# Hydr10n/DirectX-Raytracing-Spheres-Demo

Hardware: AMD Instinct MI355X
Metric: Mrays/s (CastRay-equivalents incl. primaries) at 1920x1080, 8 bounces, 1 spp (higher is better)
Workload: dtype f32

## Files before the change

### directx-raytracing-spheres-demo_amd/csrc/pt_api.hip

```cpp
#include <hip/hip_runtime.h>
#include <rccl/rccl.h>
#include <dlfcn.h>
#include <link.h>

#include <algorithm>
#include <chrono>
#include <cmath>
#include <cstdio>
#include <cstdlib>
#include <cstring>
#include <new>
#include <string>
#include <limits>
#include <vector>

#include "../../include/pt_api.h"
#include "pt_kernels.h"
#include "pt_beam_cache.h"
#include "pt_bloom.h"
#include "pt_nrd.h"
#include "pt_denoise.h"
#include "pt_lbvh.h"
#include "pt_lbvh_gpu.h"

using namespace pt;

namespace {

constexpr uint32_t kMaxLdsBytes = 160u * 1024u;
constexpr uint32_t kSahMaxSpheres = 4096u;
constexpr uint32_t kLdsSceneBudget = 64u * 1024u;

struct EventPair {
    hipEvent_t a, b;
    int kind;
};

}

struct Knobs {
    int split = -1, traverse_blocks_per_cu = -1, fused_threads = -1, no_adaptive_grid = -1, shade_blocks_per_cu = -1, tail_threshold = -1,
        tail_blocks_per_cu = -1, loop_threads = -1, inline2_min_slots = -1, tail_after = -1, seg = -1, loop_use_tail = -1, fuse_loop = -1,
        ray_replacement = -1, dyn_blocks_per_cu = -1, debug_counts = -1, sah = -1, sah_max_spheres = -1, beams = -1, wide = -1, descent = -1, roctx = -1, lane_priority = -1, fused_refit = -1, beam_reach = -1, beam_max_slack_pct = -1, beam_max_margin = -1, beam_share_wgs = -1, refl_beams = -1;
};

struct Lane {
    hipStream_t stream = nullptr;
    hipEvent_t ev_done = nullptr;
    size_t cap_slots = 0;
    RayQueue q[2]{};
    Scratch scratch{};
    bool scratch_spp = false;
    uint32_t* d_counts = nullptr;
    size_t cap_counts = 0;
    uint32_t parity = 0;
    uint32_t* h_counts = nullptr;
    uint32_t* h_prev_counts = nullptr;
    uint32_t* d_prev_counts = nullptr;
    uint64_t prev_signature = 0;
    uint32_t* d_seg_counts = nullptr;
    static constexpr uint32_t kTotals = 10;
    unsigned long long* d_totals = nullptr;
    float4* d_sph = nullptr;
    float4* d_sph_sorted = nullptr;
    float4* d_nodes = nullptr;
    uint32_t* d_refit_flags = nullptr;
    uint32_t* d_refit_hdr = nullptr;
    PtSphere* h_stage = nullptr;
    const float4* d_stage = nullptr;
    hipEvent_t ev_upload = nullptr;
    hipEvent_t ev_poll[4] = {};
    uint32_t scene_n = 0;
    bool scene_private = false;
    uint64_t sph_gen = 0;
    bool needs_refit = false;
    bool upload_pending = false;
    const void* last_out = nullptr;
    const void* last_dn[3] = {};
    const void* last_di[2] = {};
    float4* d_rot = nullptr;
    float4* h_rot_stage = nullptr;
    hipEvent_t ev_rot = nullptr;
    uint64_t rot_gen = 0;
    uint32_t rot_n = 0;
    float4* d_prev_pose = nullptr;
    float4* h_prev_stage = nullptr;
    hipEvent_t ev_prev = nullptr;
    uint32_t prev_cap = 0;
    hipEvent_t ev_gb_in = nullptr;
    void* last_gb[13] = {};
};
constexpr uint32_t kMaxLanes = 8;

struct PtContext {
    int device = 0;
    hipStream_t stream = nullptr;
// ... 364 lines not shown
    sv.nodes = priv ? L->d_nodes : c->d_nodes;
    sv.wide = priv ? nullptr : c->d_wide;
    sv.sph_sorted = priv ? L->d_sph_sorted : c->d_sph_sorted;
    sv.sorted_id = c->d_leaf_ids ? c->d_leaf_ids : c->d_sorted_id;
    sv.alpha_class = c->d_alpha_class;
    sv.alpha_tested = c->alpha_tested ? 1u : 0u;
    sv.sph = priv ? L->d_sph : c->d_sph;
    sv.mats = c->d_mats;
    sv.n = c->n;
    sv.n_nodes = c->n_nodes;
    sv.stack_depth = stack_entries(c, sv.wide != nullptr);
    sv.descent_cap = c->lds_scene ? 0u : knob_or(c->knobs.descent, 8u);
    sv.lds_scene = c->lds_scene ? 1u : 0u;
    for (int i = 0; i < 4; i++) sv.env[i] = c->sd.EnvironmentLightColor[i];
    if (c->has_textures) { sv.tex = c->d_tex; sv.tex_maps = c->d_tex_maps; sv.rot = (c->rot_gen != c->rot_master_gen && L && L->d_rot && L->rot_gen == c->rot_gen) ? L->d_rot : c->d_rot; }
    sv.env_tex = c->sd.EnvironmentLightTextureDescriptor;
    sv.env_cube = c->sd.IsEnvironmentLightTextureCubeMap ? 1u : 0u;
    for (int r = 0; r < 3; r++)
        for (int k = 0; k < 3; k++) sv.env_xf[3 * r + k] = c->sd.EnvironmentLightTransform[4 * r + k];
    sv.lights = c->d_lights; sv.n_lights = c->n_lights;
    return sv;
}

FrameParams make_frame_params(const PtContext* c)
{
    FrameParams fp{};
    fp.cam = camera_params(c->cam, c->gs.RenderSize[0], c->gs.RenderSize[1]);
    fp.frame_index = c->gs.FrameIndex;
    fp.bounces = c->gs.Bounces;
    fp.spp = c->gs.SamplesPerPixel;
    fp.rr_enabled = c->gs.IsRussianRouletteEnabled ? 1u : 0u;
    fp.throughput_threshold = c->gs.ThroughputThreshold;
    fp.inv_spp = 1.0f / (float)c->gs.SamplesPerPixel;
    fp.di_enabled = (c->gs.IsDIEnabled && c->n_lights > 0) ? 1u : 0u;
    return fp;
}

int env_knob(const char* name)
{
    const char* v = std::getenv(name);
    if (!v || !*v) return -1;
    return (int)std::strtoul(v, nullptr, 10);
}

Knobs read_knobs()
{
    Knobs k;
    k.split = env_knob("PT_SPLIT"); k.traverse_blocks_per_cu = env_knob("PT_TRAVERSE_BLOCKS_PER_CU"); k.fused_threads = env_knob("PT_FUSED_THREADS");
    k.no_adaptive_grid = std::getenv("PT_NO_ADAPTIVE_GRID") ? 1 : -1; k.shade_blocks_per_cu = env_knob("PT_SHADE_BLOCKS_PER_CU");
    k.tail_threshold = env_knob("PT_TAIL_THRESHOLD"); k.tail_blocks_per_cu = env_knob("PT_TAIL_BLOCKS_PER_CU"); k.loop_threads = env_knob("PT_LOOP_THREADS");
    k.inline2_min_slots = env_knob("PT_INLINE2_MIN_SLOTS"); k.tail_after = env_knob("PT_TAIL_AFTER"); k.seg = env_knob("PT_SEG");
    k.loop_use_tail = std::getenv("PT_LOOP_USE_TAIL") ? 1 : -1; k.fuse_loop = env_knob("PT_FUSE_LOOP"); k.beam_reach = env_knob("PT_BEAM_REACH"); k.beam_max_slack_pct = env_knob("PT_BEAM_MAX_SLACK_PCT"); k.beam_max_margin = env_knob("PT_BEAM_MAX_MARGIN"); k.beam_share_wgs = env_knob("PT_BEAM_SHARE_WGS"); k.lane_priority = env_knob("PT_LANE_PRIORITY"); k.fused_refit = env_knob("PT_FUSED_REFIT"); k.ray_replacement = env_knob("PT_RAY_REPLACEMENT");
    k.dyn_blocks_per_cu = env_knob("PT_DYN_BLOCKS_PER_CU"); k.debug_counts = std::getenv("PT_DEBUG_COUNTS") ? 1 : -1; k.sah = env_knob("PT_SAH");
    k.sah_max_spheres = env_knob("PT_SAH_MAX_SPHERES"); k.beams = env_knob("PT_BEAMS"); k.refl_beams = env_knob("PT_REFL_BEAMS"); k.wide = env_knob("PT_WIDE"); k.descent = env_knob("PT_DESCENT"); k.roctx = env_knob("PT_ROCTX");
    return k;
}

EventPair* next_events(PtContext* c, int kind)
{
    if (c->ev_used >= (1u << 20)) return nullptr;
    if (c->ev_used == c->ev_pool.size()) {
        EventPair p{};
        if (hipEventCreate(&p.a) != hipSuccess || hipEventCreate(&p.b) != hipSuccess) return nullptr;
        c->ev_pool.push_back(p);
    }
    EventPair* p = &c->ev_pool[c->ev_used++];
    p->kind = kind;
    return p;
}

uint64_t bytes_per_secondary(bool split) { return split ? 144ull : 96ull; }
uint64_t fixed_bytes(bool split, uint64_t slots, uint64_t pixels, uint64_t spp_paths)
{
    return (split ? 112ull * slots : 0ull) + 16ull * pixels + 48ull * spp_paths;
}

FrameCounters make_counters(const Lane& L, uint32_t parity)
{
    FrameCounters fc{};
    fc.counts = L.d_counts + (size_t)parity * 2 * L.cap_counts;
    fc.fold_counts = L.d_counts + (size_t)(parity ^ 1u) * 2 * L.cap_counts;
    fc.n_counts = (uint32_t)L.cap_counts - 1u;
    fc.tail_rays = L.d_totals + 2 + parity;
    fc.fold_tail = L.d_totals + 2 + (parity ^ 1u);
    fc.totals = L.d_totals;
    fc.host_counts = L.d_prev_counts;
    return fc;
}

hipError_t flush_all_counters(Lane& L)
{
    if (!L.d_counts) return hipSuccess;
    for (uint32_t i = 0; i < 2; i++) {
        const FrameCounters fc = make_counters(L, L.parity ^ 1u ^ i);
        hipError_t e = launch_flush_counters(fc.counts, fc.n_counts, fc.tail_rays, fc.totals, fc.host_counts, L.stream);
        if (e != hipSuccess) return e;
    }
    return hipSuccess;
}

void sum_events(PtContext* c, size_t begin, size_t end, PtStats* stats)
{
    for (size_t i = begin; i < end; i++) {
        float t = 0;
        if (hipEventElapsedTime(&t, c->ev_pool[i].a, c->ev_pool[i].b) != hipSuccess) continue;
        switch (c->ev_pool[i].kind) {
            case 2: stats->ms_shade += t; stats->shade_launches++; break;
// ... 312 lines not shown
    c->next_lane = (c->next_lane + 1) % c->n_lanes;
    c->frames++;
    const uint32_t* beam_lists = nullptr;
    const uint32_t* refl_lists = nullptr;
    BeamJob beam_job{};
    if (!split && !L.scene_private && c->n_nodes > 0 && knob_or(c->knobs.beams, 1u) != 0 && std::fabs(c->cam.Jitter[0]) <= 0.5f && std::fabs(c->cam.Jitter[1]) <= 0.5f) {
        hipEvent_t beam_wait = nullptr;
        if ((st = beam_cache_lookup(c, pm, std::min(primary_grid, knob_or(c->knobs.beam_share_wgs, 128u)) * 64u, &beam_lists, &refl_lists, &beam_wait, &beam_job)) != PT_OK) return st;
        if (beam_wait) PT_HIP(c, hipStreamWaitEvent(L.stream, beam_wait, 0));
    } else {
        c->beam.last_key.clear();
        c->beam.inc.active = false;
    }
    if (L.stream != c->stream) {
        const uint64_t nl = c->n_lanes;
        PT_HIP(c, hipEventRecord(c->ev_in[c->calls % nl], c->stream));
        const hipEvent_t marker = c->ev_in[c->calls >= nl - 1 ? (c->calls - (nl - 1)) % nl : 0];
        if (hipEventQuery(marker) != hipSuccess) {
            (void)hipGetLastError();
            PT_HIP(c, hipStreamWaitEvent(L.stream, marker, 0));
        }
        const void* mine[4] = { out, dn ? dn->diffuse : nullptr, dn ? dn->specular : nullptr, dn ? dn->spec_hit_dist : nullptr };
        bool reused = false;
        for (uint32_t i = 0; i < c->n_lanes && !reused; i++) {
            if (&c->lanes[i] == &L) continue;
            const Lane& o = c->lanes[i];
            const void* theirs[6] = { o.last_out, o.last_dn[0], o.last_dn[1], o.last_dn[2], o.last_di[0], o.last_di[1] };
            for (int a = 0; a < 4 && !reused; a++)
                for (int b = 0; b < 6 && !reused; b++) reused = mine[a] && mine[a] == theirs[b];
        }
        if (ext) reused = true;
        if (reused) PT_HIP(c, hipStreamWaitEvent(L.stream, c->ev_in[c->calls % nl], 0));
        L.last_out = out;
        for (int a = 0; a < 3; a++) L.last_dn[a] = mine[a + 1];
        L.last_di[0] = ext ? ext->diffuse : nullptr;
        L.last_di[1] = ext ? ext->specular : nullptr;
        c->calls++;
    }

    const SceneView sv = make_scene_view(c, &L);
    Scratch scr = L.scratch;
    scr.dn = DenoiseOut{};
    if (dn) {
        scr.dn = *dn;
        scr.dn.rec = L.scratch.dn.rec;
        scr.dn.di_s = L.scratch.dn.di_s;
    }
    FrameParams fp = make_frame_params(c);
    if (ext) fp.di_enabled = kDiExternal;
    fp.beam_lists = beam_lists;
    fp.beam_job = beam_job;
    fp.refl_lists = refl_lists;
    L.parity ^= 1u;
    const FrameCounters fc = make_counters(L, L.parity);
    uint32_t* counts = fc.counts;

    const uint64_t signature = ((uint64_t)pm.n_slots << 32) ^ ((uint64_t)bounces << 20) ^ ((uint64_t)spp << 4) ^ pm.mode ^ ((uint64_t)c->n << 40) ^ (split ? 8u : 0u);
    const bool have_prev = spp == 1 && L.prev_signature == signature && L.h_prev_counts[0] == pm.n_slots && c->knobs.no_adaptive_grid < 0;
    auto estimate = [&](size_t k) -> uint32_t {
        if (!have_prev || k >= L.cap_counts) return pm.n_slots;
        const uint64_t e = (uint64_t)L.h_prev_counts[k] + L.h_prev_counts[k] / 4 + 64;
        return (uint32_t)std::min<uint64_t>(e, pm.n_slots);
    };
    const uint32_t trav_cap_wide = c->num_cus * 8u;
    const uint32_t shade_cap = c->num_cus * knob_or(c->knobs.shade_blocks_per_cu, 16);
    const bool loop_is_main = spp > 1 && !split && c->knobs.tail_threshold < 0;
    const uint32_t tail_cap = c->num_cus * knob_or(c->knobs.tail_blocks_per_cu, loop_is_main ? 2 : 8);
    const uint32_t trav_threads = traverse_threads(c->lds_scene);
    const uint32_t loop_threads = knob_or(c->knobs.loop_threads, c->lds_scene && (loop_is_main || big_frame) ? 512u : 256u);
    const bool inline2 = !split && spp == 1 && pm.n_slots >= knob_or(c->knobs.inline2_min_slots, 0u);
    const size_t tail_after = knob_or(c->knobs.tail_after, split ? 4 : (inline2 ? 0 : 1));
    const uint32_t tail_threshold = knob_or(c->knobs.tail_threshold, 262144);

    const bool timed = stats != nullptr;
    const size_t ev_begin = c->ev_used;
    if (timed) PT_HIP(c, hipEventRecord(c->ev0, L.stream));

    auto bracket = [&](int kind, auto&& launch) -> hipError_t {
        EventPair* ev = c->profiling ? next_events(c, kind) : nullptr;
        if (ev) (void)hipEventRecord(ev->a, L.stream);
        hipError_t e = launch();
        if (ev) (void)hipEventRecord(ev->b, L.stream);
        return e;
    };
    auto poll = [&](size_t k, bool& empty, bool& go_loop) -> PtStatus {
        empty = false;
        if (loop_is_main) {
            go_loop = true;
        } else if (spp > 1) {
            constexpr size_t kPollLag = 2;
            PT_HIP(c, hipMemcpyAsync(L.h_counts + k + 1, counts + k + 1, sizeof(uint32_t), hipMemcpyDeviceToHost, L.stream));
            PT_HIP(c, hipEventRecord(L.ev_poll[k & 3], L.stream));
            go_loop = k + 2 >= wf_cap;
            if (k >= kPollLag) {
                PT_HIP(c, hipEventSynchronize(L.ev_poll[(k - kPollLag) & 3]));
                const uint32_t v = L.h_counts[k - kPollLag + 1];
                empty = v == 0;
                go_loop = go_loop || v < tail_threshold;
            }
        } else {
            go_loop = k >= tail_after || k + 2 >= wf_cap;
        }
        return PT_OK;
    };

    auto submit = [&]() -> PtStatus {
        if (ext) {
// ... 1344 lines not shown
```

### directx-raytracing-spheres-demo_amd/csrc/pt_device.h

```cpp
#pragma once

#include <hip/hip_runtime.h>
#include <stdint.h>

#include "pt_bsdf.h"
#include "pt_texture.h"
#include "pt_surface.h"
#include "pt_light.h"

namespace pt {

struct RayQueue {
    float4* q0;
    float4* q1;
    float4* q2;
    uint2* hit;
};

constexpr uint32_t kFlagBounceMask = 0xFFu;
constexpr uint32_t kFlagSampleShift = 8;
constexpr uint32_t kFlagSampleMask = 0xFFFFu;
constexpr uint32_t kFlagDirty = 1u << 24;
constexpr uint32_t kFlagViaTransmission = 1u << 25;
constexpr uint32_t kFlagDnSpecular = 1u << 26;
// ... 73 lines not shown
        const uint32_t bpt_shift = m.ts_shift - 3u;
        const uint32_t b = w >> 6, l = w & 63u;
        const uint32_t lx = ((b & ((1u << bpt_shift) - 1u)) << 3) + (l & 7u), ly = ((b >> bpt_shift) << 3) + (l >> 3);
        uint32_t gt;
        if (m.run == 1u) {
            gt = m.first + k * m.stride;
        } else {
            const uint32_t q = fast_div(k, m.run, m.inv_run, m.exact_div != 0);
            gt = m.first + q * m.stride + (k - q * m.run);
        }
        const uint32_t ty = fast_div(gt, m.tiles_x, m.inv_tiles_x, m.exact_div != 0), tx = gt - ty * m.tiles_x;
        r.px = (tx << m.ts_shift) + lx;
        r.py = (ty << m.ts_shift) + ly;
        r.valid = gt < m.tiles_total && r.px < m.img_w && r.py < m.img_h;
        r.out_index = (k << ts2_shift) + (ly << m.ts_shift) + lx;
    }
    return r;
}

struct BeamJob {
    uint32_t* lists;
    uint32_t first_block, n_blocks;
    float centre[3];
    float slack;
    float right[3], up[3], forward[3];
    float margin_px;
};

struct FrameParams {
    CameraParams cam;
    uint32_t frame_index, bounces, spp, rr_enabled;
    float throughput_threshold;
    float inv_spp;
    uint32_t di_enabled;
    const uint32_t* beam_lists;
    BeamJob beam_job;
    const uint32_t* refl_lists;
};

constexpr uint32_t kDiExternal = 2u;

struct FrameCounters {
    uint32_t* counts;
    uint32_t* fold_counts;
    uint32_t n_counts;
    unsigned long long* tail_rays;
    unsigned long long* fold_tail;
    unsigned long long* totals;
    uint32_t* host_counts;
    uint32_t* seg_counts;
    uint32_t n_segs;
    uint32_t seg_cap;
    uint32_t fuse_loop;
};

constexpr uint32_t kMaxSegs = 2048;

struct DenoiseOut {
    uint32_t mode;
    float4* rec;
    float4* di_s;
    float4* diffuse;
    float4* specular;
    float* spec_hit_dist;
};

struct Scratch {
    float4* sample_rad;
    float4* radiance;
    uint2* primary_hit;
    float4* di;
    float4* primary_cache;
    DenoiseOut dn;
};

}
```

### directx-raytracing-spheres-demo_amd/csrc/pt_trace.h

```cpp
#pragma once

#include "pt_kernels.h"
#include "pt_beam.h"

namespace pt {

__device__ __forceinline__ uint32_t lane_id() { return __builtin_amdgcn_mbcnt_hi(~0u, __builtin_amdgcn_mbcnt_lo(~0u, 0u)); }

__device__ __forceinline__ float fast_rcp(float x) { return __builtin_amdgcn_rcpf(x); }

__device__ __forceinline__ float slab_rcp(float d)
{
    const float kTiny = 1e-30f;
    return fast_rcp(__builtin_fabsf(d) < kTiny ? __builtin_copysignf(kTiny, d) : d);
}

__device__ __forceinline__ void block_atomic_add(unsigned long long* counter, unsigned long long v)
{
    __shared__ unsigned long long s_part[16];
#pragma unroll
    for (int off = 32; off > 0; off >>= 1) v += __shfl_down(v, off, 64);
    __syncthreads();
    if ((threadIdx.x & 63u) == 0) s_part[threadIdx.x >> 6] = v;
    __syncthreads();
// ... 184 lines not shown
                stack[sp] = stack_encode<StackT>(far_c);
                sp += stride;
                node = near_c;
            } else if (h0) {
                node = c0;
            } else if (h1) {
                node = c1;
            } else if (sp == 0) {
                node = kTraversalDone;
            } else {
                sp -= stride;
                node = stack_decode(stack[sp]);
            }
            if (--budget == 0u) break;
        }
        if (node == kTraversalDone) break;
        if (node >= 0) continue;
        {
            if (kCount) n_spheres_tested++;
            const uint32_t k = ~(uint32_t)node;
            const float4 s = sph[k];
            float t;
            if (intersect_sphere(o, d, tmin, kInf, make_f3(s.x, s.y, s.z), s.w, t)) {
                const uint32_t idf = ids[k];
                if ((idf >> kIdClassShift) == 0u || alpha_candidate<kAlphaTex>(sv, idf, make_f3(s.x, s.y, s.z), s.w, o, d, t)) {
                    const uint32_t id = idf & kIdMask;
                    if (t < best || (t == best && best_id != kMissId && id < best_id)) { best = t; best_id = id; }
                }
            }
        }
        if (sp == 0) break;
        sp -= stride;
        node = stack_decode(stack[sp]);
    }
    t_out = best; id_out = best_id;
    if (kCount && visits) { visits[0] += n_nodes_visited; visits[1] += n_spheres_tested; }
}

template <bool kLds, typename StackT, bool kAlphaTex = false>
__device__ __forceinline__ void closest_hit_any(const SceneView& sv, const float4* __restrict__ nodes, const float4* __restrict__ sph,
                                                const uint32_t* __restrict__ ids, f3 o, f3 d, float tmin, float tmax, StackT* stack, uint32_t stride,
                                                float& t_out, uint32_t& id_out, uint32_t* visits = nullptr)
{
    if (!kLds && visits) {
        if (sv.wide) closest_hit<StackT, true, true, kAlphaTex>(sv, sv.wide, sph, ids, sv.n, o, d, tmin, tmax, stack, stride, t_out, id_out, visits, sv.descent_cap);
        else closest_hit<StackT, true, false, kAlphaTex>(sv, nodes, sph, ids, sv.n, o, d, tmin, tmax, stack, stride, t_out, id_out, visits, sv.descent_cap);
    } else if (!kLds && sv.wide) {
        closest_hit<StackT, false, true, kAlphaTex>(sv, sv.wide, sph, ids, sv.n, o, d, tmin, tmax, stack, stride, t_out, id_out, nullptr, sv.descent_cap);
    } else {
        closest_hit<StackT, false, false, kAlphaTex>(sv, nodes, sph, ids, sv.n, o, d, tmin, tmax, stack, stride, t_out, id_out, nullptr, sv.descent_cap);
    }
}

__device__ __forceinline__ void flush_visit_counters(unsigned long long* totals, const uint32_t v[2])
{
    block_atomic_add(totals + 6, v[0]);
    block_atomic_add(totals + 7, v[1]);
}


template <typename StackT>
__device__ __forceinline__ void beam_walk_block(const SceneView& sv, const float4* nodes, const uint32_t* ids, StackT* stack, uint32_t stride, const PixelMap& pm,
                                                const CameraParams& cam, float slack, float margin_px, uint32_t tile, uint32_t* __restrict__ lists)
{
    uint32_t* rec = lists + (size_t)tile * kBeamRecord;
    const PixelRef pr = slot_to_pixel(pm, tile << 6);
    uint32_t count = 0;
    if (pr.valid) {
        const Beam b = make_beam(cam, pr.px, pr.py, slack, margin_px);
        if (sv.n == 1) {
            rec[1] = ids[0];
            count = 1;
        } else {
            int node = 0;
            uint32_t sp = 0;
            for (;;) {
                if (node >= 0) {
                    const float4 n0 = nodes[node * 4 + 0], n1 = nodes[node * 4 + 1], n2 = nodes[node * 4 + 2], n3 = nodes[node * 4 + 3];
                    const f3 lo0 = make_f3(n0.x, n0.y, n0.z), hi0 = make_f3(n0.w, n1.x, n1.y), lo1 = make_f3(n1.z, n1.w, n2.x), hi1 = make_f3(n2.y, n2.z, n2.w);
                    const int c0 = __builtin_bit_cast(int, n3.x), c1 = __builtin_bit_cast(int, n3.y);
                    const bool h0 = c0 >= 0 ? beam_meets_box(b, lo0, hi0) : (beam_meets_box(b, lo0, hi0) && beam_meets_leaf(b, lo0, hi0));
                    const bool h1 = c1 >= 0 ? beam_meets_box(b, lo1, hi1) : (beam_meets_box(b, lo1, hi1) && beam_meets_leaf(b, lo1, hi1));
                    if (h0 && h1) { stack[sp] = stack_encode<StackT>(c1); sp += stride; node = c0; continue; }
                    if (h0) { node = c0; continue; }
                    if (h1) { node = c1; continue; }
                } else {
                    if (count < kBeamListCap) rec[1 + count] = ids[~(uint32_t)node];
                    if (++count > kBeamListCap) break;
                }
                if (sp == 0) break;
                sp -= stride;
                node = stack_decode(stack[sp]);
            }
        }
    }
    rec[0] = count;
}

__device__ __forceinline__ bool refl_region(const SceneView& sv, const CameraParams& cam, uint32_t px, uint32_t py, const uint32_t* __restrict__ beam, uint32_t count,
                                            ReflRegion& g)
{
    f3 c[4];
    beam_corners(cam, px, py, 0.0f, c);
    f3 dir[5];
    float t[5];
    for (int k = 0; k < 4; k++) dir[k] = normalize(c[k]);
// ... 387 lines not shown
        if (pending) {
            regenerate();
        } else if (id == kMissId) {
            if (shade_miss()) return kShadeDone;
            if (finish_sample()) return kShadeDone;
            regenerate();
        }
        shade_surface();
        if (!end_sample) { spawn(); return kShadeRay; }
        return finish_sample() ? kShadeDone : kShadePending;
    }
    for (;;) {
        if (id == kMissId) { if (shade_miss()) return kShadeDone; }
        else shade_surface();
        if (!end_sample) { spawn(); return kShadeRay; }
        if (finish_sample()) return kShadeDone;
        regenerate();
    }
}

template <bool kMulti, bool kTex = false, bool kDI = false, int kCacheMode = 0, bool kDn = false, typename TraceFn = NoTrace>
__device__ __forceinline__ bool shade_step(const SceneView& sv, const PixelMap& pm, const FrameParams& fp, const Scratch& scratch,
                                           float4* __restrict__ out, PathState& ps, float t, uint32_t id, TraceFn&& trace = NoTrace(), uint32_t* di_rays = nullptr)
{
    return shade_step_ex<kMulti, kTex, kDI, kCacheMode, false, kDn>(sv, pm, fp, scratch, out, ps, t, id, false, trace, di_rays) == kShadeRay;
}

template <bool kDn = false>
__device__ __forceinline__ PathState load_path(const RayQueue& q, uint32_t i)
{
    const float4 a = q.q0[i], b = q.q1[i], c = q.q2[i];
    PathState ps;
    ps.o = load3(a); ps.d = load3(b); ps.T = load3(c);
    ps.slot = as_uint(a.w); ps.rng = as_uint(b.w);
    const uint32_t flags = as_uint(c.w);
    ps.bounce = flags & kFlagBounceMask;
    ps.sample = (flags >> kFlagSampleShift) & kFlagSampleMask;
    ps.dirty = (flags & kFlagDirty) != 0;
    ps.via_t = (flags & kFlagViaTransmission) != 0;
    ps.dn_spec = kDn && (flags & kFlagDnSpecular) != 0;
    return ps;
}

template <bool kDn = false>
__device__ __forceinline__ void store_path(const RayQueue& q, uint32_t j, const PathState& ps)
{
    const uint32_t flags = (ps.bounce & kFlagBounceMask) | ((ps.sample & kFlagSampleMask) << kFlagSampleShift) | (ps.dirty ? kFlagDirty : 0u)
                           | (ps.via_t ? kFlagViaTransmission : 0u) | (kDn && ps.dn_spec ? kFlagDnSpecular : 0u);
    q.q0[j] = make_float4(ps.o.x, ps.o.y, ps.o.z, as_float(ps.slot));
    q.q1[j] = make_float4(ps.d.x, ps.d.y, ps.d.z, as_float(ps.rng));
    q.q2[j] = make_float4(ps.T.x, ps.T.y, ps.T.z, as_float(flags));
}

constexpr uint32_t kStaticLdsMargin = (kMaxSegs + 64u) * 4u;

struct BounceArgHead { SceneView sv; PixelMap pm; FrameParams fp; };
template <typename T>
__device__ __forceinline__ T cold_arg(uint32_t offset)
{
    const __attribute__((address_space(4))) char* p = (const __attribute__((address_space(4))) char*)__builtin_amdgcn_kernarg_segment_ptr();
    asm volatile("" : "+s"(p));
    T v;
    __builtin_memcpy(&v, p + offset, sizeof(T));
    return v;
}

template <bool kLds, typename StackT, bool kPrimary, bool kLoop, bool kMulti, bool kTex, bool kInline2, bool kFuse, bool kDI, bool kDn>
__global__ __launch_bounds__(kFusedThreads) __attribute__((amdgpu_waves_per_eu(4, 4))) void bounce_kernel(SceneView sv, PixelMap pm, FrameParams fp, RayQueue qin, RayQueue qout,
                                                               Scratch scratch, float4* __restrict__ out,
                                                               const uint32_t* __restrict__ count_in_ptr, uint32_t* __restrict__ count_out_ptr,
                                                               FrameCounters fc)
{
    constexpr uint32_t kIters = (kPrimary && !kLoop && !kMulti && kInline2) ? 2u : 1u;
    if (kLoop && !kMulti && !kPrimary) __builtin_amdgcn_s_setprio(3);
    extern __shared__ float4 smem[];
    __shared__ uint32_t s_wave_count[kFusedThreads / 64];
    __shared__ uint32_t s_block_base;
    __shared__ uint32_t s_seg_count;
    __shared__ uint32_t s_seg_next;
    __shared__ uint32_t s_loop_next;
    __shared__ uint32_t s_seg_prefix[kMaxSegs + 1];
    __shared__ uint32_t s_refl[2];
    if (kPrimary && blockIdx.x == 0) frame_counters_begin(fc, pm.n_slots);
    const bool seg_out = kPrimary && !kLoop && fc.seg_counts != nullptr;
    const bool seg_in = !kPrimary && kLoop && fc.seg_counts != nullptr;
    uint32_t count;
    if (seg_in) {
        const uint32_t per = (fc.n_segs + blockDim.x - 1u) / blockDim.x;
        const uint32_t first = threadIdx.x * per;
        uint32_t sum = 0;
        for (uint32_t j = 0; j < per; j++) if (first + j < fc.n_segs) sum += fc.seg_counts[first + j];
        uint32_t incl = sum;
#pragma unroll
        for (int off = 1; off < 64; off <<= 1) { const uint32_t v = __shfl_up(incl, off, 64); if ((int)lane_id() >= off) incl += v; }
        if (lane_id() == 63u) s_wave_count[threadIdx.x >> 6] = incl;
        __syncthreads();
        uint32_t base = 0;
        for (uint32_t w = 0; w < (threadIdx.x >> 6); w++) base += s_wave_count[w];
        uint32_t run = base + incl - sum;
        for (uint32_t j = 0; j < per; j++)
            if (first + j < fc.n_segs) { s_seg_prefix[first + j] = run; run += fc.seg_counts[first + j]; }
        if (threadIdx.x == blockDim.x - 1u) s_seg_prefix[fc.n_segs] = base + incl;
        __syncthreads();
        count = s_seg_prefix[fc.n_segs];
        if (blockIdx.x == 0 && threadIdx.x == 0) *const_cast<uint32_t*>(count_in_ptr) = count;
    } else {
        count = kPrimary ? pm.n_slots : *count_in_ptr;
    }
    if (seg_out && threadIdx.x == 0) { s_seg_count = 0; s_seg_next = 0; s_loop_next = 0; }
    if (kIters > 1u && threadIdx.x == 0) { s_refl[0] = 0; s_refl[1] = 0; }
    if (blockIdx.x * blockDim.x >= count) {
        if (seg_out && threadIdx.x == 0) fc.seg_counts[blockIdx.x] = 0;
        return;
    }
    if ((seg_out || kIters > 1u) && !kLds) __syncthreads();
    const float4* nodes = sv.nodes;
    const float4* sph = sv.sph_sorted;
    const uint32_t* ids = sv.sorted_id;
    StackT* stack;
    if (kLds) {
        stage_scene(sv, smem);
        nodes = smem;
        sph = smem + sv.n_nodes * 4u;
        ids = reinterpret_cast<const uint32_t*>(smem + sv.n_nodes * 4u + sv.n);
        stack = reinterpret_cast<StackT*>(reinterpret_cast<char*>(smem) + scene_lds_bytes(sv.n_nodes, sv.n));
    } else {
        stack = reinterpret_cast<StackT*>(smem);
    }
    stack += threadIdx.x;
    const uint32_t lane = lane_id();
    const uint32_t wave = threadIdx.x >> 6;
    uint32_t my_rays = 0;
    if (kPrimary && !kLoop && wave == 0) {
        const BeamJob job = cold_arg<BeamJob>(offsetof(BounceArgHead, fp) + offsetof(FrameParams, beam_job));
        const uint32_t j = blockIdx.x * 64u + lane;
        if (j < job.n_blocks) {
            CameraParams cam_b = cold_arg<CameraParams>(offsetof(BounceArgHead, fp) + offsetof(FrameParams, cam));
            cam_b.Position = make_f3(job.centre[0], job.centre[1], job.centre[2]);
            cam_b.Right = make_f3(job.right[0], job.right[1], job.right[2]);
            cam_b.Up = make_f3(job.up[0], job.up[1], job.up[2]);
            cam_b.Forward = make_f3(job.forward[0], job.forward[1], job.forward[2]);
            beam_walk_block<StackT>(sv, nodes, ids, stack, blockDim.x, cold_arg<PixelMap>(offsetof(BounceArgHead, pm)), cam_b, job.slack, job.margin_px, job.first_block + j, job.lists);
        }
    }
    uint32_t* const cursor = const_cast<uint32_t*>(count_in_ptr) + fc.n_counts + 1u;
    for (uint32_t base = blockIdx.x * blockDim.x;; base += gridDim.x * blockDim.x) {
        uint32_t i;
        if (seg_in) {
            uint32_t b;
            const uint32_t static_end = kMulti ? 0u : gridDim.x * blockDim.x;
            if (!kMulti && base < static_end) {
                b = base + wave * 64u;
            } else {
                if (!kMulti && static_end >= count) break;
                uint32_t v = 0;
                if (lane == 0) v = atomicAdd(cursor, 64u);
                b = static_end + __builtin_amdgcn_readfirstlane(v);
            }
            if (b >= count) break;
            i = b + lane;
        } else if (seg_out) {
            uint32_t w = 0;
            if (lane == 0) w = atomicAdd(&s_seg_next, 1u);
            w = __builtin_amdgcn_readfirstlane(w);
            const uint32_t waves = blockDim.x >> 6;
            const uint32_t b = (blockIdx.x + (w / waves) * gridDim.x) * blockDim.x;
            if (b >= count) break;
            i = b + (w % waves) * 64u + lane;
        } else {
            if (base >= count) break;
            i = base + threadIdx.x;
        }
        bool emit = false;
        PathState ps;
        const uint32_t* beam_rec = nullptr;
        uint32_t beam_count = ~0u;
        if (kPrimary && fp.beam_lists) {
            beam_rec = fp.beam_lists + (size_t)__builtin_amdgcn_readfirstlane(i >> 6) * kBeamRecord;
            beam_count = __builtin_amdgcn_readfirstlane(beam_rec[0]);
        }
        if (i < count) {
            bool live = true;
            float tmin = 0.0f, tmax = kInf;
            if (kPrimary) {
                const PixelMap pm_c = cold_arg<PixelMap>(offsetof(BounceArgHead, pm));
                const PixelRef pr = slot_to_pixel(pm_c, i);
                live = pr.valid;
                ps.slot = i; ps.bounce = 0; ps.sample = 0; ps.dirty = false; ps.via_t = false; ps.dn_spec = false; ps.rng = 0;
                ps.T = make_f3(1.f, 1.f, 1.f);
                ps.o = make_f3(0.f, 0.f, 0.f); ps.d = make_f3(0.f, 0.f, 1.f);
                if (live) {
                    const CameraParams cam_c = cold_arg<CameraParams>(offsetof(BounceArgHead, fp) + offsetof(FrameParams, cam));
                    primary_ray(cam_c, pr.px, pr.py, ps.o, ps.d, tmin, tmax);
                    ps.rng = rng_init(pr.px, pr.py, fp.frame_index);
                } else if (pm_c.mode == 1) {
                    out[pr.out_index] = make_float4(0.f, 0.f, 0.f, 0.f);
                }
            } else if (seg_in) {
                uint32_t lo = 0, hi = fc.n_segs;
                while (hi - lo > 1u) { const uint32_t mid = (lo + hi) >> 1; if (s_seg_prefix[mid] <= i) lo = mid; else hi = mid; }
                ps = load_path<kDn>(qin, lo * fc.seg_cap + (i - s_seg_prefix[lo]));
            } else {
                ps = load_path<kDn>(qin, i);
            }
            constexpr bool kMerged = kLoop && kMulti && !kPrimary;
            if (kMerged) {
                constexpr int kCacheMode = kTex ? 0 : 2;
                bool pending = false;
                for (;;) {
                    float t = 0.0f;
                    uint32_t id = kMissId;
                    if (!pending) closest_hit_any<kLds, StackT, kTex>(sv, nodes, sph, ids, ps.o, ps.d, 0.0f, kInf, stack, blockDim.x, t, id);
                    const int r = shade_step_ex<true, kTex, false, kCacheMode, true, kDn>(sv, pm, fp, scratch, out, ps, t, id, pending);
                    if (r == kShadeDone) break;
                    pending = r == kShadePending;
                    if (!pending) my_rays++;
                }
            } else if (live) {
                bool primary_trace = kPrimary;
                uint32_t iter = 0;
                for (;;) {
                    float t;
                    uint32_t id;
                    if (kPrimary && primary_trace && fp.beam_lists && beam_count <= kBeamListCap) {
                        closest_hit_list<kTex>(sv, beam_rec, beam_count, ps.o, ps.d, tmin, tmax, t, id);
                        if (kMulti) scratch.primary_hit[i] = make_uint2(as_uint(t), id);
                    } else {
// ... 14 lines not shown
                    constexpr int kCacheMode = (kMulti && !kTex) ? ((kPrimary && !kLoop) ? 1 : ((kLoop && !kPrimary) ? 2 : 0)) : 0;
                    if (kDI)
                        emit = shade_step<kMulti, kTex, true, kCacheMode, kDn>(sv, pm, fp, scratch, out, ps, t, id,
                                                              [&](f3 so, f3 sd, float& t2, uint32_t& id2) { closest_hit_any<kLds, StackT, kTex>(sv, nodes, sph, ids, so, sd, 0.0f, kInf, stack, blockDim.x, t2, id2); },
                                                              &my_rays);
                    else
                        emit = shade_step<kMulti, kTex, false, kCacheMode, kDn>(sv, pm, fp, scratch, out, ps, t, id);
                    if (!emit) break;
                    if (!kLoop && ++iter >= kIters) break;
                    my_rays++;
                    tmin = 0.0f; tmax = kInf;
                }
            }
        }
        if (seg_out) {
            const unsigned long long mask = __ballot(emit);
            const uint32_t wave_n = __popcll(mask);
            uint32_t base = 0;
            if (lane == 0 && wave_n) base = atomicAdd(&s_seg_count, wave_n);
            base = __shfl(base, 0, 64);
            if (emit) store_path<kDn>(qout, blockIdx.x * fc.seg_cap + base + __popcll(mask & ((1ull << lane) - 1ull)), ps);
        } else if (!kLoop) {
            const unsigned long long mask = __ballot(emit);
            const uint32_t wave_n = __popcll(mask);
            const uint32_t prefix = __popcll(mask & ((1ull << lane) - 1ull));
            if (lane == 0) s_wave_count[wave] = wave_n;
            __syncthreads();
            if (threadIdx.x == 0) {
                uint32_t total = 0;
                const uint32_t n_waves = blockDim.x >> 6;
                for (uint32_t w = 0; w < n_waves; w++) { const uint32_t c = s_wave_count[w]; s_wave_count[w] = total; total += c; }
                s_block_base = total ? atomicAdd(count_out_ptr, total) : 0u;
            }
            __syncthreads();
            if (emit) store_path<kDn>(qout, s_block_base + s_wave_count[wave] + prefix, ps);
            __syncthreads();
        }
    }
    uint32_t my_loop_rays = 0;
    if (seg_out) {
        __syncthreads();
        const uint32_t n_own = s_seg_count;
        if (threadIdx.x == 0) {
            fc.seg_counts[blockIdx.x] = n_own;
            if (kFuse && n_own) atomicAdd(count_out_ptr, n_own);
        }
        if (kFuse) {
            for (;;) {
                uint32_t w = 0;
                if (lane == 0) w = atomicAdd(&s_loop_next, 64u);
                w = __builtin_amdgcn_readfirstlane(w);
                if (w >= n_own) break;
                const uint32_t i = w + lane;
                if (i < n_own) {
                    PathState ps = load_path<kDn>(qout, blockIdx.x * fc.seg_cap + i);
                    for (;;) {
                        float t;
                        uint32_t id;
                        closest_hit_any<kLds, StackT, kTex>(sv, nodes, sph, ids, ps.o, ps.d, 0.0f, kInf, stack, blockDim.x, t, id);
                        if (!shade_step<kMulti, kTex, false, 0, kDn>(sv, pm, fp, scratch, out, ps, t, id)) break;
                        my_loop_rays++;
                    }
                }
            }
        }
    }
    if (kLoop || kIters > 1u || kFuse || kDI) {
        unsigned long long total = my_rays, total2 = kFuse ? my_loop_rays : 0u;
#pragma unroll
        for (int off = 32; off > 0; off >>= 1) {
            total += __shfl_down(total, off, 64);
            if (kFuse) total2 += __shfl_down(total2, off, 64);
        }
        __shared__ uint32_t s_wave_count2[kFusedThreads / 64];
        __syncthreads();
        if (lane == 0) { s_wave_count[wave] = (uint32_t)total; if (kFuse) s_wave_count2[wave] = (uint32_t)total2; }
        __syncthreads();
        if (threadIdx.x == 0) {
            unsigned long long sum = 0, sum2 = 0;
            for (uint32_t w = 0; w < (blockDim.x >> 6); w++) { sum += s_wave_count[w]; if (kFuse) sum2 += s_wave_count2[w]; }
            if (sum + sum2) atomicAdd(fc.tail_rays, sum + sum2);
            if (sum && !kLoop && !kDI) atomicAdd(fc.totals + 4, sum);
            if (kIters > 1u && s_refl[0]) { atomicAdd(fc.totals + 8, (unsigned long long)s_refl[0]); if (s_refl[1]) atomicAdd(fc.totals + 9, (unsigned long long)s_refl[1]); }
        }
    }
}

template <bool kLds, typename StackT>
hipError_t launch_bounce_for(const SceneView& sv, const PixelMap& pm, const FrameParams& fp, const RayQueue& qin, const RayQueue& qout,
                             const Scratch& scratch, float4* out, const uint32_t* count_in, uint32_t* count_out, const FrameCounters& fc,
                             bool primary, bool loop, bool inline2, uint32_t threads, uint32_t grid, hipStream_t stream)
{
    const uint32_t lds = (sv.lds_scene ? scene_lds_bytes(sv.n_nodes, sv.n) : 0u) + threads * sv.stack_depth * (uint32_t)sizeof(StackT);
#define PT_BOUNCE9(P, LP, M, X, I, F, D, N)                                                                                \
    do {                                                                                                                    \
        if (lds + kStaticLdsMargin > 65536u) (void)hipFuncSetAttribute((const void*)bounce_kernel<kLds, StackT, P, LP, M, X, I, F, D, N>, hipFuncAttributeMaxDynamicSharedMemorySize, (int)lds); \
        hipLaunchKernelGGL((bounce_kernel<kLds, StackT, P, LP, M, X, I, F, D, N>), dim3(grid), dim3(threads), lds, stream, sv, pm, fp, qin, qout, scratch, out, count_in, count_out, fc); \
    } while (0)
#define PT_BOUNCE8(P, LP, M, X, I, F, D)                                                                                   \
    do { if (scratch.dn.mode) PT_BOUNCE9(P, LP, M, X, I, F, D, true); else PT_BOUNCE9(P, LP, M, X, I, F, D, false); } while (0)
#define PT_BOUNCE7(P, LP, M, X, I, F)                                                                                      \
    do { if (fp.di_enabled && fp.di_enabled != kDiExternal && P && !LP) PT_BOUNCE8(P, LP, M, X, I, F, (P && !LP)); else PT_BOUNCE8(P, LP, M, X, I, F, false); } while (0)
#define PT_BOUNCE6(P, LP, M, X, I)                                                                                         \
    do { if (fc.fuse_loop && P && !LP) PT_BOUNCE7(P, LP, M, X, I, (P && !LP)); else PT_BOUNCE7(P, LP, M, X, I, false); } while (0)
#define PT_BOUNCE5(P, LP, M, X)                                                                                            \
    do { if (inline2 && P && !LP && !M) PT_BOUNCE6(P, LP, M, X, (P && !LP && !M)); else PT_BOUNCE6(P, LP, M, X, false); } while (0)
#define PT_BOUNCE4(P, LP, M)                                                                                               \
// ... 23 lines not shown
```

Before: 42520.

## Add cooperative multi-lane BVH walk for sparse waves in tail bounce loops

Once fewer than half of a wave's lanes still have live paths in the loop and fused tail kernels, each surviving ray is spread across groups of 2, 4 or 8 lanes. Each lane in a group starts traversal from a different subtree of a precomputed BVH cut held in LDS, and lanes share the closest hit through DPP min reductions. This targets divergence and idle lanes in later bounces, where the path count per wave drops. In exchange it adds shuffle, ballot and reduction overhead, redundant sphere tests across subtrees, and extra LDS for the cut. It is on by default and can be turned off with the PT_COOP_WALK knob.

```diff
diff --git a/directx-raytracing-spheres-demo_amd/csrc/pt_api.hip b/directx-raytracing-spheres-demo_amd/csrc/pt_api.hip
--- a/directx-raytracing-spheres-demo_amd/csrc/pt_api.hip
+++ b/directx-raytracing-spheres-demo_amd/csrc/pt_api.hip
@@ -41,7 +41,7 @@
 struct Knobs {
     int split = -1, traverse_blocks_per_cu = -1, fused_threads = -1, no_adaptive_grid = -1, shade_blocks_per_cu = -1, tail_threshold = -1,
         tail_blocks_per_cu = -1, loop_threads = -1, inline2_min_slots = -1, tail_after = -1, seg = -1, loop_use_tail = -1, fuse_loop = -1,
-        ray_replacement = -1, dyn_blocks_per_cu = -1, debug_counts = -1, sah = -1, sah_max_spheres = -1, beams = -1, wide = -1, descent = -1, roctx = -1, lane_priority = -1, fused_refit = -1, beam_reach = -1, beam_max_slack_pct = -1, beam_max_margin = -1, beam_share_wgs = -1, refl_beams = -1;
+        ray_replacement = -1, dyn_blocks_per_cu = -1, debug_counts = -1, sah = -1, sah_max_spheres = -1, beams = -1, wide = -1, descent = -1, roctx = -1, lane_priority = -1, fused_refit = -1, beam_reach = -1, beam_max_slack_pct = -1, beam_max_margin = -1, beam_share_wgs = -1, refl_beams = -1, coop_walk = -1;
 };
 
 struct Lane {
@@ -512,7 +512,7 @@
     k.inline2_min_slots = env_knob("PT_INLINE2_MIN_SLOTS"); k.tail_after = env_knob("PT_TAIL_AFTER"); k.seg = env_knob("PT_SEG");
     k.loop_use_tail = std::getenv("PT_LOOP_USE_TAIL") ? 1 : -1; k.fuse_loop = env_knob("PT_FUSE_LOOP"); k.beam_reach = env_knob("PT_BEAM_REACH"); k.beam_max_slack_pct = env_knob("PT_BEAM_MAX_SLACK_PCT"); k.beam_max_margin = env_knob("PT_BEAM_MAX_MARGIN"); k.beam_share_wgs = env_knob("PT_BEAM_SHARE_WGS"); k.lane_priority = env_knob("PT_LANE_PRIORITY"); k.fused_refit = env_knob("PT_FUSED_REFIT"); k.ray_replacement = env_knob("PT_RAY_REPLACEMENT");
     k.dyn_blocks_per_cu = env_knob("PT_DYN_BLOCKS_PER_CU"); k.debug_counts = std::getenv("PT_DEBUG_COUNTS") ? 1 : -1; k.sah = env_knob("PT_SAH");
-    k.sah_max_spheres = env_knob("PT_SAH_MAX_SPHERES"); k.beams = env_knob("PT_BEAMS"); k.refl_beams = env_knob("PT_REFL_BEAMS"); k.wide = env_knob("PT_WIDE"); k.descent = env_knob("PT_DESCENT"); k.roctx = env_knob("PT_ROCTX");
+    k.sah_max_spheres = env_knob("PT_SAH_MAX_SPHERES"); k.beams = env_knob("PT_BEAMS"); k.refl_beams = env_knob("PT_REFL_BEAMS"); k.coop_walk = env_knob("PT_COOP_WALK"); k.wide = env_knob("PT_WIDE"); k.descent = env_knob("PT_DESCENT"); k.roctx = env_knob("PT_ROCTX");
     return k;
 }
 
@@ -931,7 +931,8 @@
     fp.beam_job = beam_job;
     fp.refl_lists = refl_lists;
     L.parity ^= 1u;
-    const FrameCounters fc = make_counters(L, L.parity);
+    FrameCounters fc = make_counters(L, L.parity);
+    fc.coop_walk = knob_or(c->knobs.coop_walk, 1u) != 0 ? 1u : 0u;
     uint32_t* counts = fc.counts;
 
     const uint64_t signature = ((uint64_t)pm.n_slots << 32) ^ ((uint64_t)bounces << 20) ^ ((uint64_t)spp << 4) ^ pm.mode ^ ((uint64_t)c->n << 40) ^ (split ? 8u : 0u);
diff --git a/directx-raytracing-spheres-demo_amd/csrc/pt_device.h b/directx-raytracing-spheres-demo_amd/csrc/pt_device.h
--- a/directx-raytracing-spheres-demo_amd/csrc/pt_device.h
+++ b/directx-raytracing-spheres-demo_amd/csrc/pt_device.h
@@ -149,6 +149,7 @@
     uint32_t n_segs;
     uint32_t seg_cap;
     uint32_t fuse_loop;
+    uint32_t coop_walk;
 };
 
 constexpr uint32_t kMaxSegs = 2048;
diff --git a/directx-raytracing-spheres-demo_amd/csrc/pt_trace.h b/directx-raytracing-spheres-demo_amd/csrc/pt_trace.h
--- a/directx-raytracing-spheres-demo_amd/csrc/pt_trace.h
+++ b/directx-raytracing-spheres-demo_amd/csrc/pt_trace.h
@@ -260,6 +260,147 @@
     }
 }
 
+
+constexpr uint32_t kCutSlots = 16;
+__device__ __forceinline__ void build_cut(const float4* __restrict__ nodes, int* s_cut)
+{
+    auto expand = [&](int ref, int& a, int& b) {
+        if (ref >= 0) {
+            const float4 n3 = nodes[ref * 4 + 3];
+            a = __builtin_bit_cast(int, n3.x); b = __builtin_bit_cast(int, n3.y);
+        } else {
+            a = ref; b = kTraversalDone;
+        }
+    };
+    expand(0, s_cut[0], s_cut[1]);
+    for (uint32_t k = 2; k <= 4; k <<= 1)
+        for (uint32_t j = 0; j < k; j++) expand(s_cut[k - 2 + j], s_cut[2 * k - 2 + 2 * j], s_cut[2 * k - 2 + 2 * j + 1]);
+}
+
+template <int kCtrl> __device__ __forceinline__ uint32_t dpp_u32(uint32_t v) { return (uint32_t)__builtin_amdgcn_update_dpp((int)v, (int)v, kCtrl, 0xF, 0xF, false); }
+template <int kCtrl> __device__ __forceinline__ float dpp_f32(float v) { return as_float(dpp_u32<kCtrl>(as_uint(v))); }
+constexpr int kDppSwap1 = 0xB1;
+constexpr int kDppSwap2 = 0x4E;
+constexpr int kDppMirror8 = 0x141;
+
+__device__ __forceinline__ float group_min(float v, uint32_t k)
+{
+    v = raw_minf(v, dpp_f32<kDppSwap1>(v));
+    if (k >= 4u) v = raw_minf(v, dpp_f32<kDppSwap2>(v));
+    if (k >= 8u) v = raw_minf(v, dpp_f32<kDppMirror8>(v));
+    return v;
+}
+
+template <typename StackT>
+__device__ __forceinline__ void closest_hit_coop(const float4* __restrict__ nodes, const float4* __restrict__ sph, const uint32_t* __restrict__ ids,
+                                                 const int* __restrict__ s_cut, unsigned long long ballot, f3 o, f3 d, float tmin, float tmax,
+                                                 StackT* stack, uint32_t stride, float& t_out, uint32_t& id_out, uint32_t descent_cap = 0)
+{
+    const uint32_t lane = lane_id();
+    const uint32_t n_live = (uint32_t)__builtin_amdgcn_readfirstlane(__popcll(ballot));
+    const uint32_t shift = n_live <= 8u ? 3u : (n_live <= 16u ? 2u : 1u), k = 1u << shift;
+    const uint32_t group = lane >> shift, j = lane & (k - 1u);
+    uint32_t src;
+    {
+        const uint32_t lo = (uint32_t)ballot, hi = (uint32_t)(ballot >> 32);
+        uint32_t r = group, m = lo, c = __popc(lo);
+        src = 0;
+        if (r >= c) { r -= c; m = hi; src = 32u; }
+#pragma unroll
+        for (uint32_t w = 16; w > 0; w >>= 1) {
+            c = __popc(m & ((1u << w) - 1u));
+            if (r >= c) { r -= c; m >>= w; src += w; }
+        }
+    }
+    const bool has_ray = group < n_live;
+    src = has_ray ? src : lane;
+    const f3 ro = make_f3(__shfl(o.x, (int)src, 64), __shfl(o.y, (int)src, 64), __shfl(o.z, (int)src, 64));
+    const f3 rd = make_f3(__shfl(d.x, (int)src, 64), __shfl(d.y, (int)src, 64), __shfl(d.z, (int)src, 64));
+    const float rtmin = __shfl(tmin, (int)src, 64), rtmax = __shfl(tmax, (int)src, 64);
+    const float ix = slab_rcp(rd.x), iy = slab_rcp(rd.y), iz = slab_rcp(rd.z);
+    const float ox = -ro.x * ix, oy = -ro.y * iy, oz = -ro.z * iz;
+    float best = rtmax;
+    float cull = rtmax;
+    uint32_t best_id = kMissId;
+    int node = has_ray ? s_cut[k - 2u + j] : kTraversalDone;
+    uint32_t sp = 0;
+    for (;;) {
+        uint32_t budget = descent_cap;
+        while (node >= 0) {
+            const float4 n0 = nodes[node * 4 + 0];
+            const float4 n1 = nodes[node * 4 + 1];
+            const float4 n2 = nodes[node * 4 + 2];
+            const float4 n3 = nodes[node * 4 + 3];
+            const float ax = pt_fma(n0.x, ix, ox), bx = pt_fma(n0.w, ix, ox);
+            const float ay = pt_fma(n0.y, iy, oy), by = pt_fma(n1.x, iy, oy);
+            const float az = pt_fma(n0.z, iz, oz), bz = pt_fma(n1.y, iz, oz);
+            const float lx0 = fminf(ax, bx); const float cx = pt_fma(n1.z, ix, ox);
+            const float ly0 = fminf(ay, by); const float dx = pt_fma(n2.y, ix, ox);
+            const float lz0 = fminf(az, bz); const float cy = pt_fma(n1.w, iy, oy);
+            const float hx0 = fmaxf(ax, bx); const float dy = pt_fma(n2.z, iy, oy);
+            const float hy0 = fmaxf(ay, by); const float cz = pt_fma(n2.x, iz, oz);
+            const float hz0 = fmaxf(az, bz); const float dz = pt_fma(n2.w, iz, oz);
+            const float tn0 = fmaxf(fmaxf(lx0, ly0), raw_maxf(lz0, rtmin));
+            const float tf0 = fminf(fminf(hx0, hy0), raw_minf(hz0, cull));
+            const float tn1 = fmaxf(fmaxf(fminf(cx, dx), fminf(cy, dy)), raw_maxf(fminf(cz, dz), rtmin));
+            const float tf1 = fminf(fminf(fmaxf(cx, dx), fmaxf(cy, dy)), raw_minf(fmaxf(cz, dz), cull));
+            const bool h0 = tn0 <= tf0, h1 = tn1 <= tf1;
+            const int c0 = __builtin_bit_cast(int, n3.x), c1 = __builtin_bit_cast(int, n3.y);
+            if (h0 && h1) {
+                const bool swap = tn1 < tn0;
+                const int near_c = swap ? c1 : c0, far_c = swap ? c0 : c1;
+                stack[sp] = stack_encode<StackT>(far_c);
+                sp += stride;
+                node = near_c;
+            } else if (h0) {
+                node = c0;
+            } else if (h1) {
+                node = c1;
+            } else if (sp == 0) {
+                node = kTraversalDone;
+            } else {
+                sp -= stride;
+                node = stack_decode(stack[sp]);
+            }
+            if (--budget == 0u) break;
+        }
+        if (node < 0 && node != kTraversalDone) {
+            const uint32_t q = ~(uint32_t)node;
+            const float4 s = sph[q];
+            float t;
+            if (intersect_sphere(ro, rd, rtmin, kInf, make_f3(s.x, s.y, s.z), s.w, t)) {
+                const uint32_t idf = ids[q];
+                if ((idf >> kIdClassShift) != kAlphaInvisible) {
+                    const uint32_t id = idf & kIdMask;
+                    if (t < best || (t == best && best_id != kMissId && id < best_id)) { best = t; best_id = id; }
+                }
+            }
+            if (sp == 0) {
+                node = kTraversalDone;
+            } else {
+                sp -= stride;
+                node = stack_decode(stack[sp]);
+            }
+        }
+        cull = group_min(raw_minf(cull, best), k);
+        if (__ballot(node != kTraversalDone) == 0ull) break;
+    }
+#define PT_COOP_MERGE(CTRL)                                                                                              \
+    {                                                                                                                    \
+        const float t2 = dpp_f32<CTRL>(best);                                                                            \
+        const uint32_t id2 = dpp_u32<CTRL>(best_id);                                                                     \
+        if (t2 < best || (t2 == best && id2 < best_id)) { best = t2; best_id = id2; }                                    \
+    }
+    PT_COOP_MERGE(kDppSwap1)
+    if (k >= 4u) PT_COOP_MERGE(kDppSwap2)
+    if (k >= 8u) PT_COOP_MERGE(kDppMirror8)
+#undef PT_COOP_MERGE
+    const uint32_t rank = __popcll(ballot & ((1ull << lane) - 1ull));
+    const int owner = (int)((rank << shift) & 63u);
+    t_out = __shfl(best, owner, 64);
+    id_out = __shfl(best_id, owner, 64);
+}
+
 __device__ __forceinline__ void flush_visit_counters(unsigned long long* totals, const uint32_t v[2])
 {
     block_atomic_add(totals + 6, v[0]);
@@ -753,7 +894,7 @@
     q.q2[j] = make_float4(ps.T.x, ps.T.y, ps.T.z, as_float(flags));
 }
 
-constexpr uint32_t kStaticLdsMargin = (kMaxSegs + 64u) * 4u;
+constexpr uint32_t kStaticLdsMargin = (kMaxSegs + 64u + kCutSlots) * 4u;
 
 struct BounceArgHead { SceneView sv; PixelMap pm; FrameParams fp; };
 template <typename T>
@@ -764,6 +905,28 @@
     T v;
     __builtin_memcpy(&v, p + offset, sizeof(T));
     return v;
+}
+
+template <typename StackT, bool kDn>
+__device__ __forceinline__ void coop_bounces(const SceneView& sv, const PixelMap& pm, const FrameParams& fp, const Scratch& scratch, float4* __restrict__ out,
+                                             const float4* __restrict__ nodes, const float4* __restrict__ sph, const uint32_t* __restrict__ ids,
+                                             const int* __restrict__ s_cut, StackT* stack, uint32_t stride, PathState& ps, bool alive, uint32_t& rays)
+{
+    for (;;) {
+        const unsigned long long ballot = __ballot(alive);
+        if (ballot == 0ull) break;
+        float t = 0.0f;
+        uint32_t id = kMissId;
+        if (__popcll(ballot) > 32) {
+            if (alive) closest_hit<StackT, false, false, false>(sv, nodes, sph, ids, sv.n, ps.o, ps.d, 0.0f, kInf, stack, stride, t, id, nullptr, sv.descent_cap);
+        } else {
+            closest_hit_coop<StackT>(nodes, sph, ids, s_cut, ballot, ps.o, ps.d, 0.0f, kInf, stack, stride, t, id, sv.descent_cap);
+        }
+        if (alive) {
+            alive = shade_step<false, false, false, 0, kDn>(sv, pm, fp, scratch, out, ps, t, id);
+            if (alive) rays++;
+        }
+    }
 }
 
 template <bool kLds, typename StackT, bool kPrimary, bool kLoop, bool kMulti, bool kTex, bool kInline2, bool kFuse, bool kDI, bool kDn>
@@ -782,6 +945,8 @@
     __shared__ uint32_t s_loop_next;
     __shared__ uint32_t s_seg_prefix[kMaxSegs + 1];
     __shared__ uint32_t s_refl[2];
+    __shared__ int s_cut[kCutSlots];
+    constexpr bool kCoop = kLds && !kMulti && !kTex && !kDI && !kDn && sizeof(StackT) == 2 && ((kLoop && !kPrimary) || kFuse);
     if (kPrimary && blockIdx.x == 0) frame_counters_begin(fc, pm.n_slots);
     const bool seg_out = kPrimary && !kLoop && fc.seg_counts != nullptr;
     const bool seg_in = !kPrimary && kLoop && fc.seg_counts != nullptr;
@@ -825,12 +990,17 @@
         sph = smem + sv.n_nodes * 4u;
         ids = reinterpret_cast<const uint32_t*>(smem + sv.n_nodes * 4u + sv.n);
         stack = reinterpret_cast<StackT*>(reinterpret_cast<char*>(smem) + scene_lds_bytes(sv.n_nodes, sv.n));
+        if (kCoop && fc.coop_walk != 0u && sv.n > 1u) {
+            if (threadIdx.x == 0) build_cut(smem, s_cut);
+            __syncthreads();
+        }
     } else {
         stack = reinterpret_cast<StackT*>(smem);
     }
     stack += threadIdx.x;
     const uint32_t lane = lane_id();
     const uint32_t wave = threadIdx.x >> 6;
+    const bool coop = kCoop && fc.coop_walk != 0u && sv.n > 1u && (blockDim.x & 63u) == 0u;
     uint32_t my_rays = 0;
     if (kPrimary && !kLoop && wave == 0) {
         const BeamJob job = cold_arg<BeamJob>(offsetof(BounceArgHead, fp) + offsetof(FrameParams, beam_job));
@@ -874,6 +1044,22 @@
         }
         bool emit = false;
         PathState ps;
+        if (kCoop && kLoop && coop) {
+            const bool alive = i < count;
+            if (alive) {
+                if (seg_in) {
+                    uint32_t lo = 0, hi = fc.n_segs;
+                    while (hi - lo > 1u) { const uint32_t mid = (lo + hi) >> 1; if (s_seg_prefix[mid] <= i) lo = mid; else hi = mid; }
+                    ps = load_path<kDn>(qin, lo * fc.seg_cap + (i - s_seg_prefix[lo]));
+                } else {
+                    ps = load_path<kDn>(qin, i);
+                }
+            } else {
+                ps.o = make_f3(0.f, 0.f, 0.f); ps.d = make_f3(0.f, 0.f, 1.f);
+            }
+            coop_bounces<StackT, kDn>(sv, pm, fp, scratch, out, nodes, sph, ids, s_cut, stack, blockDim.x, ps, alive, my_rays);
+            continue;
+        }
         const uint32_t* beam_rec = nullptr;
         uint32_t beam_count = ~0u;
         if (kPrimary && fp.beam_lists) {
@@ -994,7 +1180,12 @@
                 w = __builtin_amdgcn_readfirstlane(w);
                 if (w >= n_own) break;
                 const uint32_t i = w + lane;
-                if (i < n_own) {
+                if (kCoop && coop) {
+                    PathState ps;
+                    if (i < n_own) ps = load_path<kDn>(qout, blockIdx.x * fc.seg_cap + i);
+                    else { ps.o = make_f3(0.f, 0.f, 0.f); ps.d = make_f3(0.f, 0.f, 1.f); }
+                    coop_bounces<StackT, kDn>(sv, pm, fp, scratch, out, nodes, sph, ids, s_cut, stack, blockDim.x, ps, i < n_own, my_loop_rays);
+                } else if (i < n_own) {
                     PathState ps = load_path<kDn>(qout, blockIdx.x * fc.seg_cap + i);
                     for (;;) {
                         float t;
```

Result: faster. 43950, median of 6 (+3.4%).
